# tdavchev/DESIRE

Hardware: AMD Instinct MI355X
Metric: agent-trajectory-samples/sec (K=20, T_pred=40) (higher is better)
Workload: dtype f32; 1 GPU; BASELINE configs[1]: SDD-like synthetic windows, 32 agent slots/window, K=20, T_obs=8/T_pred=40, H=128, L=128, fp32, posterior CVAE, IOC 1 refinement, social grid 4x4, scene grid 64x64x32; 512 windows/step/GPU; windows_per_gpu=512, rows_per_gpu=327680, parallelism=scene-sharded x1

## Files before the change

### desire_amd/csrc/api.hip

```cpp
#include "ctx.h"

#include <cmath>
#include <cstdio>
#include <cstdlib>
#include <cstring>

static thread_local std::string g_err;
int desire_fail(int code, const std::string& msg) { g_err = msg; return code; }

extern "C" const char* desire_last_error(void) { return g_err.c_str(); }
extern "C" int desire_version(void) { return 5; }
extern "C" int desire_dims_size(void) { return (int)sizeof(desire_dims); }
#ifndef DESIRE_SRC_HASH
#define DESIRE_SRC_HASH "unstamped"
#endif
extern "C" const char* desire_build_hash(void) { return DESIRE_SRC_HASH; }

int desire_upload(desire_ctx* h, const std::string& name, const std::vector<float>& v) {
    const size_t bytes = v.size() * sizeof(float);
    const DevBuf* b = h->dev.find(name.c_str());
    if (!b || b->bytes != bytes) {
        h->dev.release(name.c_str());
        if (h->dev.ensure(name.c_str(), bytes)) return -1;
    }
// ... 103 lines not shown
    return 0;
}

}

extern "C" int desire_set_option(desire_handle* h, const char* name, int32_t value) {
    if (!h || !name) return fail(DESIRE_ERR_ARG, "null argument");
    desire_dims d = h->d;
    const std::string nm(name);
    if (nm == "ioc_form") d.ioc_form = value;
    else if (nm == "ioc_split") d.ioc_split = value;
    else if (nm == "train_fp32_mask") d.train_fp32_mask = value;
    else if (nm == "flags") d.flags = value;
    else if (nm == "compact_host_counts") {
        h->cp_host_counts = value != 0;
        h->cp_pending = false; h->cp_enc = false;
        return DESIRE_OK;
    }
    else if (nm == "scene_grad") {
        if (value != 0 && value != 1) return fail(DESIRE_ERR_ARG, "scene_grad must be 0 or 1");
        h->scene_grad = value != 0;
        return scene_grad_on(h) && h->training ? scene_grad_setup(h) : DESIRE_OK;
    }
    else if (nm == "compact_min_rows") {
        if (value < 0) return fail(DESIRE_ERR_ARG, "compact_min_rows must be >= 0");
        h->ci_min_rows = value;
        return DESIRE_OK;
    }
    else if (nm == "scene_modes_chunk") {
        if (value < 0) return fail(DESIRE_ERR_ARG, "scene_modes_chunk must be >= 0");
        h->scene_modes_chunk = value;
        return DESIRE_OK;
    }
    else return fail(DESIRE_ERR_ARG, "unknown option: " + nm + " (ioc_form, ioc_split, train_fp32_mask, flags, compact_min_rows, compact_host_counts, scene_grad, scene_modes_chunk)");
    if (int rc = check_options(d)) return rc;
    if (((d.flags ^ h->d.flags) & (DESIRE_FLAG_COMPACT_ROWS | DESIRE_FLAG_COMPACT_IOC)) ||
        ((d.flags & DESIRE_FLAG_COMPACT_IOC) && (d.ioc_form != h->d.ioc_form || d.train_fp32_mask != h->d.train_fp32_mask)))
        h->cp_pending = h->cp_enc = false;
    h->d = d;
    return DESIRE_OK;
}

extern "C" int desire_create(const desire_dims* dims, desire_handle** out) {
    if (!dims || !out) return fail(DESIRE_ERR_ARG, "null argument");
    if (int rc = check_dims(*dims)) return rc;
    int ndev = 0;
    if (hipGetDeviceCount(&ndev) != hipSuccess || ndev < 1)
        return fail(DESIRE_ERR_NODEV, "no HIP device: libdesire_hip has no CPU path");
    int dev = 0;
    HIPCHK(hipGetDevice(&dev));
    hipDeviceProp_t prop;
    HIPCHK(hipGetDeviceProperties(&prop, dev));
    if (std::strncmp(prop.gcnArchName, "gfx950", 6) != 0)
        return fail(DESIRE_ERR_NODEV, std::string("device is ") + prop.gcnArchName + ", kernels are built for gfx950 only");
    desire_ctx* h = new desire_ctx();
    h->d = *dims;
    h->Hl = dims->H;
    if (dims->H < 64) h->d.H = 64;
    h->A = dims->n_scenes * dims->mno;
    h->R = h->A * dims->K;
    h->V = dims->S * dims->S;
    h->B = dims->grid_size * dims->grid_size;
    h->E = dims->E_v + dims->C + h->d.H;
    pack::weight_shapes(h->d, h->d.H, h->V, h->B, h->want);
    pack::weight_shapes(h->d, h->Hl, h->V, h->B, h->want_user);
    if (h->Hl != h->d.H) embeddings(h);
    const desire_dims& d = h->d;
// ... 215 lines not shown
```

### desire_amd/csrc/api_forward.hip

```cpp
#include "ctx.h"

#include <cmath>
#include <cstdio>
#include <cstdlib>
#include <cstring>

bool compact_rows(const desire_ctx* h) { return (h->d.flags & DESIRE_FLAG_COMPACT_ROWS) != 0; }
bool compact_ioc(const desire_ctx* h) { return (h->d.flags & DESIRE_FLAG_COMPACT_IOC) && ioc_plan(h).fwd != IocFwd::STEPWISE; }
ClassLayout class_layout(const desire_ctx* h, bool pad, const int* counts) {
    const desire_dims& d = h->d;
    ClassLayout L;
    int cand[6], nc = 0;
    for (int m : {8, 10, 16, 32, 64, 96}) if (m < d.mno && (m != 10 || pad)) cand[nc++] = m;
    for (int i = nc > 3 ? nc - 3 : 0; i < nc; ++i) L.m[L.n++] = cand[i];
    L.m[L.n++] = d.mno;
    for (int i = L.n; i < 4; ++i) L.m[i] = d.mno;
    for (int c = 0; c < L.n; ++c) {
        IocView& v = L.c[c];
        v.cls = c; v.mno = L.m[c]; v.n_scenes = counts ? counts[c] : d.n_scenes;
        v.gpt = (v.mno <= 32 && 32 % v.mno) ? 32 / v.mno : 0; v.ngrp = v.n_scenes * d.K;
        v.R = v.gpt ? (long)((v.ngrp + v.gpt - 1) / v.gpt) * 32 : (long)v.ngrp * v.mno;
        v.agent_off = L.agents; v.row_off = L.rows; v.win_off = L.wins;
        L.agents += (size_t)v.n_scenes * v.mno; L.rows += (size_t)v.R; L.wins += (size_t)v.n_scenes;
    }
// ... 215 lines not shown
        }
        const int32_t* amap = Wt<const int32_t>(h, "cp_amap");
        Timer t(h, s, "compact_gather");
        if (!h->cp_enc) {
            launch_gather_agents(W(h, "HxHy"), W(h, "cp_HxHy"), amap, P, 2 * H, s, dynP);
            launch_gather_agents(W(h, "p_last"), W(h, "cp_plast"), amap, P, 2, s, dynP);
            if (d.posterior) launch_gather_agents(W(h, "params"), W(h, "cp_params"), amap, P, 2 * d.L, s, dynP);
        }
        HxS = W(h, "cp_HxHy"); plS = W(h, "cp_plast"); Yout = W(h, "cp_Y0");
    }
    if (!dev_eps) {
        Timer t(h, s, "reparam");
        if (compact) launch_reparam_c_rng(W(h, "cp_params"), rng_args(h), W(h, "z"), Wt<const int32_t>(h, "cp_amap"), mno, d.K, d.mno, d.L, d.posterior, s, dynP);
        else launch_reparam_rng(W(h, "params"), rng_args(h), W(h, "z"), R, d.L, d.K, d.mno, d.posterior, s);
    }
    else if (compact) { Timer t(h, s, "reparam"); launch_reparam_c(W(h, "cp_params"), dev_eps, W(h, "z"), Wt<const int32_t>(h, "cp_amap"), mno, d.K, d.mno, d.L, d.posterior, s, dynP); }
    else { Timer t(h, s, "reparam"); launch_reparam(W(h, "params"), dev_eps, W(h, "z"), R, d.L, d.K, d.mno, d.posterior, s); }
    auto normd = [&](const char* layer, float* x, int P, int C, int sig) { batch_stats_act(h, layer, x, R, P, C, sig, s); };
    GemmArgs g{};
    g.A = W(h, "z"); g.lda = d.L; g.M = R; g.K = d.L; g.Bp = gen_op(h, GenStage::DECONV1, plan.deconv1); g.G = d.L / 8;
    g.NT = 64; g.out = W(h, "d1"); g.ldo = 2048; g.N = 2048;
    g.p0 = D(h, "vae_dec/deconv1/scale"); g.p1 = D(h, "vae_dec/deconv1/shift"); g.chmod = 128;
    int hintS = 0;
    if (dyn) hintS = count_hint(h);
    g.dyn = DynCount{dynP, d.K, hintS}; g.M_hint = hintS * d.K;
    const bool pobn = plan.batch_stats;
    { Timer t(h, s, "deconv1");
      switch (plan.deconv1) {
          case GenForm::BF16: launch_deconv1_bf16(g, s); break;
          case GenForm::X6: launch_deconv1_x6(g, s); break;
          case GenForm::FP32: launch_gemm_rows(g, pobn ? EPI_NONE : EPI_SCALE_SHIFT_ELU, s); if (pobn) normd("vae_dec/deconv1", W(h, "d1"), 16, 128, 0);
      } }
    ConvArgs c{};
    c.n = R; c.dyn = DynCount{dynP, d.K, hintS};
    if (pobn) c.mode = 3;
    c.in = W(h, "d1"); c.out = W(h, "d2"); c.Wp = gen_op(h, GenStage::DECONV2, plan.deconv2);
    c.scale = D(h, "vae_dec/deconv2/scale"); c.shift = D(h, "vae_dec/deconv2/shift");
    { Timer t(h, s, "deconv2");
      switch (plan.deconv2) {
          case GenForm::BF16: launch_deconv2_bf16(c, s); break;
          case GenForm::X6: launch_deconv2_x6(c, s, plan.np); break;
          case GenForm::FP32: launch_deconv2(c, s); if (pobn) normd("vae_dec/deconv2", W(h, "d2"), 64, 64, 0);
      } }
    c.in = W(h, "d2"); c.out = W(h, "d3"); c.Wp = gen_op(h, GenStage::DECONV3, plan.deconv3);
    c.scale = D(h, "vae_dec/deconv3/scale"); c.shift = D(h, "vae_dec/deconv3/shift");
    const float* w4 = D(h, gen_operands(GenStage::DECONV4, plan.deconv4()).a);
    if (plan.fuse34) {
        c.w_raw = w4; c.out = W(h, "xhat");
        Timer t(h, s, "deconv34");
        launch_deconv34_bf16(c, D(h, "vae_dec/deconv4/scale"), D(h, "vae_dec/deconv4/shift"), s);
    } else {
        { Timer t(h, s, "deconv3");
          switch (plan.deconv3) {
              case GenForm::BF16: launch_deconv3_bf16(c, s); break;
              case GenForm::X6: launch_deconv3_x6(c, s, plan.np); break;
              case GenForm::FP32: launch_deconv3(c, s); if (pobn) normd("vae_dec/deconv3", W(h, "d3"), 256, 32, 0);
          } }
        c.in = W(h, "d3"); c.out = W(h, "xhat"); c.w_raw = w4;
        c.scale = D(h, "vae_dec/deconv4/scale"); c.shift = D(h, "vae_dec/deconv4/shift");
        { Timer t(h, s, "deconv4"); launch_deconv4(c, s);
          if (pobn) normd("vae_dec/deconv4", W(h, "xhat"), 1024, 1, 1); }
    }
    MaskArgs m{};
    m.xhat = W(h, "xhat"); m.R = R; m.V = h->V; m.H = H; m.Hl = h->Hl; m.K = d.K; m.mno = mno;
    m.Wp = gen_op(h, GenStage::MASK, plan.mask); m.bias = D(h, "mask/b"); m.Hx = HxS; m.ldhx = 2 * H; m.xz = W(h, "xz");
    m.dyn = DynCount{dynP, 1, hintS};
    if (h->training) m.sv_p = W(h, "mask_sv_p");
// ... 218 lines not shown
```

### desire_amd/csrc/backward.hip

```cpp
#include "ctx.h"

namespace {

float* G(desire_ctx* h, const std::string& name) { return W(h, "Gflat") + h->slots.at(name).off; }

void tn(desire_ctx* h, const float* A, int lda, const float* Gm, int ldg, long M, int Kd, int N, float* out, int ldo,
        int accumulate, hipStream_t s, const unsigned long long* flags = nullptr, int fcols = 0,
        const int* rowlist = nullptr, const int* binbase = nullptr, const int* bintotal = nullptr) {
    TnArgs a{};
    a.A = A; a.lda = lda; a.G = Gm; a.ldg = ldg; a.M = M; a.Kd = Kd; a.N = N; a.flags = flags; a.fcols = fcols;
    a.rowlist = rowlist; a.binbase = binbase; a.bintotal = bintotal;
    if (rowlist && !(fcols == 128 && N > 64 && gemm_tn_big_tiles(a) > 0)) a.rowlist = nullptr;
    if (a.rowlist) a.flags = nullptr;
    a.np = gen_plan(h).wgrad_pieces;
    const long big_tiles = a.np == 2 ? gemm_tn_big_tiles(a) : 0;
    const long blocks = ((Kd + 63) / 64) * ((N + 63) / 64);
    long sl = big_tiles ? 512 / big_tiles : 2048 / blocks;
    if (sl < 1) sl = 1; if (sl > (big_tiles ? 512 : 256)) sl = big_tiles ? 512 : 256;
    const long maxsl = (M + 63) / 64; if (sl > maxsl) sl = maxsl;
    while ((size_t)sl * Kd * N * sizeof(float) > h->ws.bytes("tn_partial") && sl > 1) sl /= 2;
    a.nslices = (int)sl; a.partial = W(h, "tn_partial");
    launch_gemm_tn(a, out, ldo, accumulate, s);
}
void colsum(desire_ctx* h, const float* Gm, int ldg, long M, int N, float* out, int accumulate, hipStream_t s) {
// ... 377 lines not shown
    launch_gemm_rows(g, EPI_NONE, s);
    return DESIRE_OK;
}

int cvae_enc_bwd(const BwdPass& bp) {
    desire_ctx* h = bp.h; hipStream_t s = bp.s; const desire_dims& d = h->d;
    const int H = d.H, V = h->V, L = d.L, Ae = bp.agents_e;
    const bool bn1 = d.bn_mode != 0;
    const int32_t* inv = bp.rows_compact ? Wt<const int32_t>(h, "cp_inv") : nullptr;
    if (bp.eps) launch_reparam_bwd(W(h, "dz"), bp.eps, W(h, "params"), bp.valid, W(h, "nvalid"), W(h, "dparams"), d.n_scenes, d.mno, d.K, L, s, inv, bp.n_present);
    else launch_reparam_bwd_rng(W(h, "dz"), rng_args(h), W(h, "params"), bp.valid, W(h, "nvalid"), W(h, "dparams"), d.n_scenes, d.mno, d.K, L, s, inv,
                                bp.n_present);
    if (bp.enc_compact) launch_gather_agents(W(h, "dparams"), W(h, "cp_dparams"), bp.amap, bp.n_present, 2 * L, s);
    const float* dparE = bp.enc_compact ? W(h, "cp_dparams") : W(h, "dparams");
    if (Ae <= 0) return DESIRE_OK;
    tn(h, W(h, "c3"), 2048, dparE, 2 * L, Ae, 2048, 2 * L, G(h, "vae_enc/fc/w"), 2 * L, 0, s);
    colsum(h, dparE, 2 * L, Ae, 2 * L, G(h, "vae_enc/fc/b"), 0, s);
    GemmArgs g{};
    g.A = dparE; g.lda = 2 * L; g.M = Ae; g.K = 2 * L; g.Bp = D4(h, "vae_enc/fc/WT"); g.G = 2 * L / 8; g.NT = 64;
    g.out = W(h, "dconvE3"); g.ldo = 2048; g.N = 2048; g.p0 = D(h, "vae_enc/conv3/scale"); g.chmod = 128; g.aux = W(h, "c3");
    if (bn1) {
        launch_gemm_rows(g, EPI_NONE, s);
        norm_bwd(bp, W(h, "dconvE3"), W(h, "conv3_pre"), W(h, "c3"), Ae, 16, 128, D(h, "vae_enc/conv3/gamma"), 0);
    } else
        launch_gemm_rows(g, EPI_ELUGRAD, s);
    const int NSL = Ae >= 2048 ? 64 : (Ae >= 256 ? 16 : 4);
    ConvWgradArgs wg{};
    wg.np = gen_plan(h).wgrad_pieces;
    wg.n = Ae; wg.partial = W(h, "tn_partial");
    wg.S = W(h, "dconvE3"); wg.Cs = 128; wg.Ps = 4; wg.Lg = W(h, "c2"); wg.Cl = 64; wg.Pl = 8; wg.stride = 1; wg.pad = 0;
    launch_conv_wgrad(wg, NSL, G(h, "vae_enc/conv3/w"), s);
    if (!bn1) colsum(h, W(h, "dconvE3"), 128, (long)Ae * 16, 128, G(h, "vae_enc/conv3/b"), 0, s);
    ConvArgs c{};
    c.n = Ae; c.mode = bn1 ? 3 : 1;
    c.in = W(h, "dconvE3"); c.out = W(h, "dconvE2"); c.Wp = D4(h, "vae_enc/conv3/Wbwd");
    c.scale = D(h, "vae_enc/conv2/scale"); c.shift = c.scale; c.yprev = W(h, "c2");
    launch_deconv2(c, s);
    if (bn1) norm_bwd(bp, W(h, "dconvE2"), W(h, "conv2_pre"), W(h, "c2"), Ae, 64, 64, D(h, "vae_enc/conv2/gamma"), 0);
    wg.S = W(h, "dconvE2"); wg.Cs = 64; wg.Ps = 8; wg.Lg = W(h, "c1"); wg.Cl = 32; wg.Pl = 16; wg.stride = 2; wg.pad = 1;
    launch_conv_wgrad(wg, NSL, G(h, "vae_enc/conv2/w"), s);
    if (!bn1) colsum(h, W(h, "dconvE2"), 64, (long)Ae * 64, 64, G(h, "vae_enc/conv2/b"), 0, s);
    c.in = W(h, "dconvE2"); c.out = W(h, "dconvE1"); c.Wp = D4(h, "vae_enc/conv2/Wbwd");
    c.scale = D(h, "vae_enc/conv1/scale"); c.shift = c.scale; c.yprev = W(h, "c1");
    launch_deconv3(c, s);
    if (bn1) norm_bwd(bp, W(h, "dconvE1"), W(h, "conv1_pre"), W(h, "c1"), Ae, 256, 32, D(h, "vae_enc/conv1/gamma"), 0);
    launch_w1ch_grad(W(h, "vae_in"), W(h, "dconvE1"), Ae, Ae < 1024 ? Ae : 1024, W(h, "tn_partial"), G(h, "vae_enc/conv1/w"), s);
    if (!bn1) colsum(h, W(h, "dconvE1"), 32, (long)Ae * 256, 32, G(h, "vae_enc/conv1/b"), 0, s);
    c.in = W(h, "dconvE1"); c.out = W(h, "dq_c"); c.w_raw = D(h, "vae_enc/conv1/raw"); c.mode = 2; c.yprev = W(h, "vae_in");
    launch_deconv4(c, s);
    tn(h, bp.Hx_e, 2 * H, W(h, "dq_c"), V, Ae, 2 * H, V, G(h, "fc_c/w"), V, 0, s);
    colsum(h, W(h, "dq_c"), V, Ae, V, G(h, "fc_c/b"), 0, s);
    g = GemmArgs{};
    g.A = W(h, "dq_c"); g.lda = V; g.M = Ae; g.K = V; g.Bp = D4(h, "fc_c/WT"); g.G = V / 8; g.NT = 2 * H / 32;
    g.out = bp.dH_e; g.ldo = 2 * H; g.N = 2 * H;
    launch_gemm_rows(g, EPI_NONE, s);
    return DESIRE_OK;
}

int assemble_dH(const BwdPass& bp) {
    desire_ctx* h = bp.h; hipStream_t s = bp.s; const desire_dims& d = h->d;
    const int H = d.H, P = bp.n_present;
    if (bp.enc_compact) {
        if (P <= 0) return DESIRE_OK;
        launch_rows_to_agents(bp.dHx_s, bp.dH_e, 2 * H, 1, P, d.K, H, s);
        if (!h->ci_last) {
            launch_fill_f32(W(h, "dHxHy_ioc"), (size_t)h->A * H, 0.f, s);
            launch_rows_to_agents(W(h, "dHx_rows"), W(h, "dHxHy_ioc"), H, d.n_scenes, d.mno, d.K, H, s);
// ... 78 lines not shown
```

### desire_amd/csrc/ctx.h

```cpp
#pragma once
#include "../../include/desire_hip.h"
#include "gen_plan.h"
#include "ioc_plan.h"
#include "kernels.h"
#include "pack.h"
#include "workspace.h"

#include <hip/hip_runtime.h>

#include <cstring>
#include <functional>
#include <map>
#include <string>
#include <vector>

int desire_fail(int code, const std::string& msg);
#define fail desire_fail
#define HIPCHK(x)                                                                                   \
    do {                                                                                            \
        hipError_t e_ = (x);                                                                        \
        if (e_ != hipSuccess)                                                                       \
            return fail(DESIRE_ERR_HIP, std::string(#x) + ": " + hipGetErrorString(e_));            \
    } while (0)

// ... 5 lines not shown
struct WSlot { size_t off; size_t n; };

struct EmbedAxis { std::vector<std::pair<int, int>> seg; };
struct Embed { EmbedAxis rows, cols; };

struct desire_ctx {
    desire_dims d;
    int Hl = 0;
    int A, R, V, B, E;
    std::map<std::string, size_t> want_user;
    std::map<std::string, Embed> emb;
    std::map<std::string, std::vector<float>> host_w;
    std::map<std::string, size_t> want;
    Workspace dev{dev_malloc, dev_free};
    Workspace ws{dev_malloc, dev_free};
    bool finalized = false;
    std::vector<void*> graphs;
    std::vector<float> bin_tab_host;
    const float* grids = nullptr;
    bool grids_set = false;
    bool profiling = false;
    void* peer_region = nullptr; size_t peer_bytes = 0; void* peer_base[8] = {nullptr, nullptr, nullptr, nullptr, nullptr, nullptr, nullptr, nullptr};
    bool peer_mapped[8] = {false, false, false, false, false, false, false, false}; int peer_rank = -1, peer_nranks = 0; bool peer_ready = false;
    int* peer_err = nullptr;
    float head_loss_w = 0.f;
    int recon_mode = 0; float recon_tau = 0.f;
    int recon_scope = 0;
    int* host_err = nullptr;
    int32_t* cp_host = nullptr; hipEvent_t cp_ev = nullptr; bool cp_pending = false; int cp_P = -1;
    int ci_cnt[4] = {0, 0, 0, 0}; bool ci_last = false; int ci_min_rows = 8192;
    bool cp_enc = false;
    bool cp_host_counts = false;
    bool cp_last = false;
    int scene_modes_chunk = 0;
    int32_t* bw_starts = nullptr; int32_t* bw_err = nullptr;
    uint32_t* rng_state = nullptr; uint32_t rng_scene_base = 0, rng_slot_base = 0;
    std::vector<Prof> prof;
    std::vector<std::string> prof_name_store;
    bool training = false;
    std::map<std::string, WSlot> slots;
    size_t n_params = 0;
    const float* last_eps = nullptr;
    int adam_t = 0;
    int n_seg = 0;
    int n_seg16 = 0;
    bool scene_grad = false;
    const float* img = nullptr; bool img_set = false;
    bool img_stale = true;
};

struct Timer {
    desire_ctx* h; hipStream_t s; bool on; size_t idx = 0;
    Timer(desire_ctx* h_, hipStream_t s_, const char* name) : h(h_), s(s_), on(h_->profiling) {
        if (!on) return;
        Prof p; p.name = name;
        (void)hipEventCreate(&p.e0); (void)hipEventCreate(&p.e1);
        (void)hipEventRecord(p.e0, s);
        idx = h->prof.size();
        h->prof.push_back(p);
    }
    ~Timer() { if (on) (void)hipEventRecord(h->prof[idx].e1, s); }
};

inline GenPlan gen_plan(const desire_ctx* h) { return gen_plan(h->d, h->training, h->V); }

inline const float* D(desire_ctx* h, const char* name) { return h->dev.get(name); }
// ... 44 lines not shown
```

### desire_amd/csrc/dyn_count.h

```cpp
#pragma once
#include <stdint.h>

struct DynCount { const int32_t* cnt; int mul; int hint; };
inline int dyn_units(int worst, const DynCount& d) {
    if (!d.cnt || d.hint <= 0) return worst;
    const long g = (long)d.hint * d.mul, want = g + g / 4 + 256;
    return (int)(want < (long)worst ? want : (long)worst);
}
```

### desire_amd/csrc/kernels.h

```cpp
#pragma once
#include <hip/hip_runtime.h>
#include <stdint.h>

#include "dyn_count.h"
#include "eval_lds.h"
#include "ioc_lds.h"

template <auto K>
inline const void* big_lds_kernel() {
    static const hipError_t once = hipFuncSetAttribute(reinterpret_cast<const void*>(K), hipFuncAttributeMaxDynamicSharedMemorySize, 160 * 1024);
    (void)once;
    return reinterpret_cast<const void*>(K);
}
template <auto K, class... Args>
inline void launch_big_lds(dim3 grid, dim3 block, size_t lds, hipStream_t s, const Args&... args) {
    (void)big_lds_kernel<K>();
    hipLaunchKernelGGL(K, grid, block, lds, s, args...);
}


enum { EPI_BIAS = 0, EPI_BIAS_RELU = 1, EPI_SCALE_SHIFT_ELU = 2, EPI_NONE = 3, EPI_ELUGRAD = 4, EPI_SIGGRAD = 5 };

struct GemmArgs {
    const float* A; int lda; int M; int K;
    const float4* Bp; int G; int NT;
    float* out; int ldo; int N;
    const float* p0; const float* p1; int chmod;
    const float* aux;
    DynCount dyn;
    int M_hint;
};
void launch_gemm_rows(const GemmArgs& a, int epi, hipStream_t s);

void launch_reparam(const float* params, const float* eps, float* z, int R, int L, int K, int mno,
                    int posterior, hipStream_t s);

struct RngArgs { const uint32_t* st; uint32_t seed_lo, seed_hi, draw; uint32_t scene_base, slot_base; };
struct RngKey { uint32_t lo, hi, draw; };
__device__ __forceinline__ RngKey rng_key(const RngArgs& g) {
    if (g.st) return RngKey{g.st[2], g.st[3], g.st[1]};
    return RngKey{g.seed_lo, g.seed_hi, g.draw};
}
void launch_rng_set(uint32_t* st, uint64_t seed, uint32_t draw, hipStream_t s);
void launch_rng_begin(uint32_t* st, hipStream_t s);
void launch_rng_fill(uint64_t seed, uint32_t stream_id, uint64_t first, int normals, void* out, uint64_t n, hipStream_t s);
void launch_reparam_rng(const float* params, const RngArgs& g, float* z, int R, int L, int K, int mno, int posterior, hipStream_t s);
void launch_reparam_c_rng(const float* params_c, const RngArgs& g, float* z, const int32_t* amap, int P, int K, int mno, int L, int posterior,
                          hipStream_t s, const int32_t* dynP = nullptr);
void launch_reparam_bwd_rng(const float* dz, const RngArgs& g, const float* params, const uint8_t* valid, const float* nvalid, float* dparams,
                            int n_scenes, int mno, int K, int L, hipStream_t s, const int32_t* inv, int P);

struct MaskArgs {
    const float* xhat; int R; int V; int H; int K; int mno;
    int Hl;
    const float4* Wp; const float* bias; const float* Hx; int ldhx; float* xz;
    float* sv_p;
    DynCount dyn;
};
void launch_mask(const MaskArgs& a, hipStream_t s);
void launch_deconv1_x6(const GemmArgs& a, hipStream_t s);
void launch_mask_x6(const MaskArgs& a, hipStream_t s);

struct ConvArgs {
    const float* in; float* out; int n;
    const float4* Wp; const float* w_raw;
    const float* scale; const float* shift;
    int mode; const float* yprev;
    DynCount dyn;
};
void launch_conv1(const ConvArgs& a, hipStream_t s);
void launch_conv2(const ConvArgs& a, hipStream_t s);
void launch_conv2_x3(const ConvArgs& a, hipStream_t s);
void launch_conv3_x3(const ConvArgs& a, hipStream_t s);
void launch_conv3(const ConvArgs& a, hipStream_t s);
void launch_deconv2(const ConvArgs& a, hipStream_t s);
void launch_deconv3(const ConvArgs& a, hipStream_t s);
void launch_deconv4(const ConvArgs& a, hipStream_t s);

struct EncArgs {
    const float* frames; int n_scenes; int T; int mno;
    float sx, sy; int H;
    const float* wx_g; const float* b_g;
    const float* wx_c; const float* b_c;
    const float4* Whg; const float4* Whc;
    float* out; int ldo;
    float* p_last;
    uint8_t* valid;
    float* sv_r; float* sv_u; float* sv_c; float* sv_h; float* sv_x;
    int n_roll; const float* w5; const float* b5;
    const float* normals; float* roll_out;
    DynCount dyn;
};
void launch_encoder(const EncArgs& a, hipStream_t s);
void launch_encoder_pair(const EncArgs& past, const EncArgs& fut, hipStream_t s);
void launch_encoder_bf16(const EncArgs& a, hipStream_t s);

struct RollArgs {
    const float* h_T; int R; int K; int mno; int H; int T;
    const float* wx_g; const float* b_g; const float* wx_c; const float* b_c; const float4* Whg; const float4* Whc;
    const float* w5; const float* b5;
    const float* normals; RngArgs g;
// ... 255 lines not shown
```

### desire_amd/csrc/kernels_conv.hip

```cpp
#include "common.h"
#include "kernels.h"
#include <type_traits>
#include <utility>

__global__ __launch_bounds__(DS_WG) void k_conv1(ConvArgs a) {
    __shared__ __attribute__((aligned(16))) float in_s[36 * 40];
    const int n = blockIdx.x, tid = threadIdx.x;
    DYN_N(a, n, n)
    for (int i = tid; i < 36 * 40; i += DS_WG) in_s[i] = 0.f;
    __syncthreads();
    for (int i = tid; i < 1024; i += DS_WG) in_s[((i >> 5) + 1) * 40 + (i & 31) + 1] = a.in[(size_t)n * 1024 + i];
    const int co = tid & 31, pg = tid >> 5;
    float wr[25];
#pragma unroll
    for (int k = 0; k < 25; ++k) wr[k] = a.w_raw[k * 32 + co];
    __syncthreads();
    const float sc = a.scale[co], sh = a.shift[co];
    for (int p = pg; p < 256; p += 8) {
        const int oy = p >> 4, ox = p & 15;
        const int base = (2 * ox) & ~3;
        const bool odd = ox & 1;
        float acc = 0.f;
#pragma unroll
        for (int ky = 0; ky < 5; ++ky) {
// ... 52 lines not shown
        ox[m] = q - oy[m] * OW;
    }
    for (int ky = 0; ky < 5; ++ky)
        for (int kx = 0; kx < 5; ++kx) {
            const float* ap[MT];
#pragma unroll
            for (int m = 0; m < MT; ++m) {
                const int iy = oy[m] * STRIDE + ky - PAD, ix = ox[m] * STRIDE + kx - PAD;
                const bool ok = iy >= 0 && iy < IW && ix >= 0 && ix < IW;
                ap[m] = (ok ? in_s + (sm[m] * IW * IW + pos(iy, ix)) * LDP : zero_row) + 4 * (lane >> 5);
            }
            mma_groups_ptr<MT>(acc, ap, a.Wp + ((size_t)((ky * 5 + kx) * NT + nt) * G) * 64 + lane, G);
        }
    const int co = nt * 32 + (lane & 31);
    const float sc = a.scale[co], sh = a.shift[co];
#pragma unroll
    for (int m = 0; m < MT; ++m)
#pragma unroll
        for (int i = 0; i < 16; ++i) {
            const int r = (mt0 + m) * 32 + acc_row(i);
            const int smp = s0 + r / PIX;
            if (smp < a.n) { const size_t ix = ((size_t)s0 * PIX + r) * CO + co; a.out[ix] = conv_epilogue(acc[m][i], sc, sh, a.mode, false, a.yprev, ix); }
        }
}
void launch_conv2(const ConvArgs& a, hipStream_t s) {
    const size_t lds = (36 + 256 * 36) * sizeof(float);
    hipLaunchKernelGGL((k_conv_gather<32, 16, 8, 2, 1, 64>), dim3(a.n), dim3(DS_WG), lds, s, a);
}
void launch_conv3(const ConvArgs& a, hipStream_t s) {
    const size_t lds = (68 + 4 * 64 * 68) * sizeof(float);
    launch_big_lds<k_conv_gather<64, 8, 4, 1, 0, 128>>(dim3((a.n + 3) / 4), dim3(DS_WG), lds, s, a);
}

template <bool FWD>
__global__ __launch_bounds__(DS_WG) void k_deconv2(ConvArgs a) {
    extern __shared__ __attribute__((aligned(16))) float out_s[];
    const int lane = lane_id(), w = wave_id();
    const int hf = w & 1, sp = w >> 1;
    asm volatile("" ::: "a255");
    DYN_N(a, n, blockIdx.x * 4)
    for (int bx = blockIdx.x; bx * 4 < a.n; bx += gridDim.x) {
        const int s0 = bx * 4 + sp * 2;
        const int c = lane & 31, hi = lane >> 5;
        float O[8][8];
    #pragma unroll
        for (int oy = 0; oy < 8; ++oy)
    #pragma unroll
            for (int ox = 0; ox < 8; ++ox) O[oy][ox] = 0.f;
        float4 af[16];
        {
            const int row = lane & 31;
            const int smp = min(s0 + ((row >> 2) & 1), a.n - 1);
            const float* src = a.in + ((size_t)smp * 16 + (row >> 3) * 4 + (row & 3)) * 128 + 4 * hi;
    #pragma unroll
            for (int g = 0; g < 16; ++g) af[g] = *reinterpret_cast<const float4*>(src + g * 8);
        }
        int woff = 0;
        asm volatile("" : "+s"(woff));
        const float4* wp = a.Wp + woff + lane;
        auto load_b = [&](float4 (&b)[8], int q) {
            const float4* bp = wp + ((size_t)((q >> 1) * 2 + hf) * 16 + (q & 1) * 8) * 64;
    #pragma unroll
            for (int g = 0; g < 8; ++g) b[g] = bp[g * 64];
        };
        float4 b[2][8];
        load_b(b[0], 0);
        f32x16 acc = zero16();
    #pragma unroll
        for (int q = 0; q < 50; ++q) {
            if (q + 1 < 50) load_b(b[(q + 1) & 1], q + 1);
            __builtin_amdgcn_sched_barrier(0);
            const float4 (&bt)[8] = b[q & 1];
            if (!(q & 1)) acc = zero16();
    #pragma unroll
            for (int g = 0; g < 8; ++g) {
                const float4 av = af[(q & 1) * 8 + g];
                acc = mfma32(av.x, bt[g].x, acc);
                acc = mfma32(av.y, bt[g].y, acc);
                acc = mfma32(av.z, bt[g].z, acc);
                acc = mfma32(av.w, bt[g].w, acc);
            }
            if (q & 1) {
                const int tap = q >> 1, ky = tap / 5, kx = tap - ky * 5;
    #pragma unroll
                for (int i = 0; i < 16; ++i) O[(i >> 2) + ky][(i & 3) + kx] = O[(i >> 2) + ky][(i & 3) + kx] + acc[i];
            }
            __builtin_amdgcn_sched_barrier(0);
        }
        float* my = out_s + (sp * 2) * 4096;
    #pragma unroll
        for (int o = 0; o < 64; ++o) my[(hi * 64 + o) * 64 + hf * 32 + c] = O[o >> 3][o & 7];
        const int er = lane >> 3, ec = hf * 32 + (lane & 7) * 4;
        const float4 sc4 = *reinterpret_cast<const float4*>(a.scale + ec), sh4 = *reinterpret_cast<const float4*>(a.shift + ec);
        for (int i = 0; i < 16; ++i) {
            const int sp_px = i * 8 + er;
            const int smp = s0 + (sp_px >> 6);
            if (smp < a.n) {
                const float4 v = *reinterpret_cast<const float4*>(my + sp_px * 64 + ec);
                const size_t ix = ((size_t)smp * 64 + (sp_px & 63)) * 64 + ec;
                float4 o;
                if (FWD) {
                    o.x = eluf_(v.x * sc4.x + sh4.x); o.y = eluf_(v.y * sc4.y + sh4.y);
                    o.z = eluf_(v.z * sc4.z + sh4.z); o.w = eluf_(v.w * sc4.w + sh4.w);
                } else {
                    o.x = conv_epilogue(v.x, sc4.x, sh4.x, a.mode, false, a.yprev, ix);
                    o.y = conv_epilogue(v.y, sc4.y, sh4.y, a.mode, false, a.yprev, ix + 1);
                    o.z = conv_epilogue(v.z, sc4.z, sh4.z, a.mode, false, a.yprev, ix + 2);
                    o.w = conv_epilogue(v.w, sc4.w, sh4.w, a.mode, false, a.yprev, ix + 3);
                }
                *reinterpret_cast<float4*>(a.out + ix) = o;
            }
        }
    }
}
void launch_deconv2(const ConvArgs& a, hipStream_t s) {
    const int ng = dyn_units(a.n, a.dyn);
    if (a.mode == 0) launch_big_lds<k_deconv2<true>>(dim3((ng + 3) / 4), dim3(DS_WG), 4 * 4096 * sizeof(float), s, a);
    else launch_big_lds<k_deconv2<false>>(dim3((ng + 3) / 4), dim3(DS_WG), 4 * 4096 * sizeof(float), s, a);
}

struct D3Chain { int py, px, ky, kx; bool first, last; };
__host__ __device__ constexpr D3Chain d3_chain(int s) {
    const int c = s < 4 ? 0 : s < 10 ? 1 : s < 16 ? 2 : 3, s0 = c == 0 ? 0 : c == 1 ? 4 : c == 2 ? 10 : 16;
    const int py = c >> 1, px = c & 1, nkx = px ? 3 : 2, n = (py ? 3 : 2) * nkx, i = s - s0;
    return D3Chain{py, px, 1 - py + 2 * (i / nkx), 1 - px + 2 * (i % nkx), i == 0, i == n - 1};
}
template <class F, int... S>
__device__ __forceinline__ void static_for_(F&& f, std::integer_sequence<int, S...>) { (f(std::integral_constant<int, S>{}), ...); }
template <int N, class F>
__device__ __forceinline__ void static_for(F&& f) { static_for_(f, std::make_integer_sequence<int, N>{}); }
template <bool FWD, int NS>
__global__ __launch_bounds__(NS * 64) void k_deconv3(ConvArgs a) {
    constexpr int LDP = 68;
    extern __shared__ __attribute__((aligned(16))) float smem[];
    float* zero_row = smem;
    float* in_s = smem + 128;
    const int lane = lane_id(), w = wave_id(), tid = threadIdx.x;
    DYN_N(a, n, blockIdx.x * NS)
    for (int bx = blockIdx.x; bx * NS < a.n; bx += gridDim.x) {
        const int s0 = bx * NS;
        int woff = 0;
        asm volatile("" : "+s"(woff));
        const float4* wp = a.Wp + woff + lane;
        auto load_b = [&](float4 (&f)[8], const D3Chain ch) __attribute__((always_inline)) {
            const float4* bp = wp + ((size_t)(ch.ky * 5 + ch.kx) * 8) * 64;
    #pragma unroll
            for (int g = 0; g < 8; ++g) f[g] = bp[g * 64];
        };
        float4 b[2][8];
        load_b(b[0], d3_chain(0));
        __builtin_amdgcn_sched_barrier(0);
        for (int i = tid; i < 128; i += NS * 64) zero_row[i] = 0.f;
        for (int i = tid; i < NS * 64 * 16; i += NS * 64) {
            const int pix = i >> 4, c4 = i & 15;
            const int smp = s0 + (pix >> 6);
            float4 v = make_float4(0.f, 0.f, 0.f, 0.f);
            if (smp < a.n) v = *reinterpret_cast<const float4*>(a.in + ((size_t)s0 * 64 + pix) * 64 + c4 * 4);
            *reinterpret_cast<float4*>(in_s + pix * LDP + c4 * 4) = v;
        }
        __syncthreads();
        const int smp = s0 + w;
        const int hi = lane >> 5;
        float4 sc[4], sh[4];
    #pragma unroll
        for (int q = 0; q < 4; ++q) {
            sc[q] = *reinterpret_cast<const float4*>(a.scale + 8 * q + 4 * hi);
            sh[q] = *reinterpret_cast<const float4*>(a.shift + 8 * q + 4 * hi);
        }
        int qy[2], qx[2];
    #pragma unroll
        for (int m = 0; m < 2; ++m) { const int q = m * 32 + (lane & 31); qy[m] = q >> 3; qx[m] = q & 7; }
        auto rows = [&](const D3Chain ch, const float* (&ap)[2]) __attribute__((always_inline)) {
            const int dy = (ch.py + 1 - ch.ky) / 2, dx = (ch.px + 1 - ch.kx) / 2;
    #pragma unroll
            for (int m = 0; m < 2; ++m) {
                const int iy = qy[m] + dy, ix = qx[m] + dx;
                const bool ok = iy >= 0 && iy < 8 && ix >= 0 && ix < 8;
                const int in_off = 128 + (w * 64 + iy * 8 + ix) * LDP, zero_off = ((w * 64 + iy * 8 + ix + 64) * LDP + 128) & 63;
                ap[m] = smem + (ok ? in_off : zero_off) + 4 * hi;
            }
        };
        const float* ap[2][2];
        rows(d3_chain(0), ap[0]);
        f32x16 acc[2];
        static_for<25>([&](auto chain_no) __attribute__((always_inline)) {
            constexpr int s = decltype(chain_no)::value;
            constexpr D3Chain ch = d3_chain(s);
            constexpr int py = ch.py, px = ch.px;
            if constexpr (s + 1 < 25) { load_b(b[(s + 1) & 1], d3_chain(s + 1)); rows(d3_chain(s + 1), ap[(s + 1) & 1]); }
            __builtin_amdgcn_sched_barrier(0);
            if constexpr (ch.first) { acc[0] = zero16(); acc[1] = zero16(); }
            const float4 (&bt)[8] = b[s & 1];
    #pragma unroll
            for (int g = 0; g < 8; ++g)
    #pragma unroll
                for (int m = 0; m < 2; ++m) {
                    const float4 av = *reinterpret_cast<const float4*>(ap[s & 1][m] + g * 8);
                    acc[m] = mfma32(bt[g].x, av.x, acc[m]);
                    acc[m] = mfma32(bt[g].y, av.y, acc[m]);
                    acc[m] = mfma32(bt[g].z, av.z, acc[m]);
                    acc[m] = mfma32(bt[g].w, av.w, acc[m]);
                    __builtin_amdgcn_sched_barrier(0);
                }
            if constexpr (ch.last) {
                if (smp < a.n) {
    #pragma unroll
                    for (int m = 0; m < 2; ++m) {
                        const int oy = 2 * qy[m] + py, ox = 2 * qx[m] + px;
                        const size_t base = ((size_t)smp * 256 + oy * 16 + ox) * 32 + 4 * hi;
    #pragma unroll
                        for (int q = 0; q < 4; ++q) {
                            const size_t ix = base + 8 * q;
                            float4 o;
                            if (FWD) {
                                o.x = eluf_(acc[m][4 * q] * sc[q].x + sh[q].x); o.y = eluf_(acc[m][4 * q + 1] * sc[q].y + sh[q].y);
                                o.z = eluf_(acc[m][4 * q + 2] * sc[q].z + sh[q].z); o.w = eluf_(acc[m][4 * q + 3] * sc[q].w + sh[q].w);
                            } else {
                                o.x = conv_epilogue(acc[m][4 * q], sc[q].x, sh[q].x, a.mode, false, a.yprev, ix);
                                o.y = conv_epilogue(acc[m][4 * q + 1], sc[q].y, sh[q].y, a.mode, false, a.yprev, ix + 1);
                                o.z = conv_epilogue(acc[m][4 * q + 2], sc[q].z, sh[q].z, a.mode, false, a.yprev, ix + 2);
                                o.w = conv_epilogue(acc[m][4 * q + 3], sc[q].w, sh[q].w, a.mode, false, a.yprev, ix + 3);
                            }
                            *reinterpret_cast<float4*>(a.out + ix) = o;
                        }
                    }
                }
            }
        });
        __syncthreads();
    }
}
void launch_deconv3(const ConvArgs& a, hipStream_t s) {
    const size_t lds = (128 + (size_t)4 * 64 * 68) * sizeof(float);
    const int ng = dyn_units(a.n, a.dyn);
    if (a.mode == 0) launch_big_lds<k_deconv3<true, 4>>(dim3((ng + 3) / 4), dim3(256), lds, s, a);
    else launch_big_lds<k_deconv3<false, 4>>(dim3((ng + 3) / 4), dim3(256), lds, s, a);
}

__global__ __launch_bounds__(DS_WG) void k_deconv4(ConvArgs a) {
    constexpr int LDP = 36;
    __shared__ __attribute__((aligned(16))) float in_s[256 * LDP];
    __shared__ __attribute__((aligned(16))) float w_s[25 * 32];
    const int n = blockIdx.x, tid = threadIdx.x, lane = lane_id(), w = wave_id();
    for (int i = tid; i < 256 * 8; i += DS_WG) {
        const int pix = i >> 3, c4 = i & 7;
        *reinterpret_cast<float4*>(in_s + pix * LDP + c4 * 4) =
            *reinterpret_cast<const float4*>(a.in + ((size_t)n * 256 + pix) * 32 + c4 * 4);
    }
    for (int i = tid; i < 800; i += DS_WG) w_s[i] = a.w_raw[i];
    __syncthreads();
    const int py = w >> 1, px = w & 1;
    const float sc = a.scale[0], sh = a.shift[0];
    for (int j = 0; j < 4; ++j) {
        const int q = j * 64 + lane;
        const int qy = q >> 4, qx = q & 15;
        float acc = 0.f;
        for (int ky = 1 - py; ky < 5; ky += 2) {
            const int iy = qy + (py + 1 - ky) / 2;
            if (iy < 0 || iy >= 16) continue;
            for (int kx = 1 - px; kx < 5; kx += 2) {
                const int ix = qx + (px + 1 - kx) / 2;
                if (ix < 0 || ix >= 16) continue;
                const float* ip = in_s + (iy * 16 + ix) * LDP;
                const float* wp = w_s + (ky * 5 + kx) * 32;
#pragma unroll
                for (int c4 = 0; c4 < 8; ++c4) {
                    const float4 x = *reinterpret_cast<const float4*>(ip + c4 * 4);
                    const float4 ww = *reinterpret_cast<const float4*>(wp + c4 * 4);
                    acc = fmaf(x.x, ww.x, acc); acc = fmaf(x.y, ww.y, acc);
// ... 54 lines not shown
```

Before: 2.622 million samples/s.

## Make deconv2/deconv3 persistent with cross-iteration prefetch of next tile

Deconv2 and deconv3 launches now cap the grid at the number of resident workgroups, queried through the occupancy API or taken from a new gen_grid_cap option, and loop over tiles with a grid stride. Inside the loop, the next tile's activations and the first weight slice are prefetched into registers during the current tile's MFMA chain. This hides global load latency across iterations and removes the per-iteration staging and __syncthreads in deconv3. In exchange it raises register pressure and changes how LDS is reused between waves, which could lower occupancy or introduce races.

```diff
diff --git a/desire_amd/csrc/api.hip b/desire_amd/csrc/api.hip
--- a/desire_amd/csrc/api.hip
+++ b/desire_amd/csrc/api.hip
@@ -159,7 +159,12 @@
         h->scene_modes_chunk = value;
         return DESIRE_OK;
     }
-    else return fail(DESIRE_ERR_ARG, "unknown option: " + nm + " (ioc_form, ioc_split, train_fp32_mask, flags, compact_min_rows, compact_host_counts, scene_grad, scene_modes_chunk)");
+    else if (nm == "gen_grid_cap") {
+        if (value < 0) return fail(DESIRE_ERR_ARG, "gen_grid_cap must be >= 0");
+        h->gen_grid_cap = value;
+        return DESIRE_OK;
+    }
+    else return fail(DESIRE_ERR_ARG, "unknown option: " + nm + " (ioc_form, ioc_split, train_fp32_mask, flags, compact_min_rows, compact_host_counts, scene_grad, scene_modes_chunk, gen_grid_cap)");
     if (int rc = check_options(d)) return rc;
     if (((d.flags ^ h->d.flags) & (DESIRE_FLAG_COMPACT_ROWS | DESIRE_FLAG_COMPACT_IOC)) ||
         ((d.flags & DESIRE_FLAG_COMPACT_IOC) && (d.ioc_form != h->d.ioc_form || d.train_fp32_mask != h->d.train_fp32_mask)))
diff --git a/desire_amd/csrc/api_forward.hip b/desire_amd/csrc/api_forward.hip
--- a/desire_amd/csrc/api_forward.hip
+++ b/desire_amd/csrc/api_forward.hip
@@ -271,7 +271,7 @@
           case GenForm::FP32: launch_gemm_rows(g, pobn ? EPI_NONE : EPI_SCALE_SHIFT_ELU, s); if (pobn) normd("vae_dec/deconv1", W(h, "d1"), 16, 128, 0);
       } }
     ConvArgs c{};
-    c.n = R; c.dyn = DynCount{dynP, d.K, hintS};
+    c.n = R; c.dyn = DynCount{dynP, d.K, hintS}; c.grid_cap = h->gen_grid_cap;
     if (pobn) c.mode = 3;
     c.in = W(h, "d1"); c.out = W(h, "d2"); c.Wp = gen_op(h, GenStage::DECONV2, plan.deconv2);
     c.scale = D(h, "vae_dec/deconv2/scale"); c.shift = D(h, "vae_dec/deconv2/shift");
diff --git a/desire_amd/csrc/backward.hip b/desire_amd/csrc/backward.hip
--- a/desire_amd/csrc/backward.hip
+++ b/desire_amd/csrc/backward.hip
@@ -433,7 +433,7 @@
     launch_conv_wgrad(wg, NSL, G(h, "vae_enc/conv3/w"), s);
     if (!bn1) colsum(h, W(h, "dconvE3"), 128, (long)Ae * 16, 128, G(h, "vae_enc/conv3/b"), 0, s);
     ConvArgs c{};
-    c.n = Ae; c.mode = bn1 ? 3 : 1;
+    c.n = Ae; c.mode = bn1 ? 3 : 1; c.grid_cap = h->gen_grid_cap;
     c.in = W(h, "dconvE3"); c.out = W(h, "dconvE2"); c.Wp = D4(h, "vae_enc/conv3/Wbwd");
     c.scale = D(h, "vae_enc/conv2/scale"); c.shift = c.scale; c.yprev = W(h, "c2");
     launch_deconv2(c, s);
diff --git a/desire_amd/csrc/ctx.h b/desire_amd/csrc/ctx.h
--- a/desire_amd/csrc/ctx.h
+++ b/desire_amd/csrc/ctx.h
@@ -61,6 +61,7 @@
     bool cp_enc = false;
     bool cp_host_counts = false;
     bool cp_last = false;
+    int gen_grid_cap = 0;
     int scene_modes_chunk = 0;
     int32_t* bw_starts = nullptr; int32_t* bw_err = nullptr;
     uint32_t* rng_state = nullptr; uint32_t rng_scene_base = 0, rng_slot_base = 0;
diff --git a/desire_amd/csrc/dyn_count.h b/desire_amd/csrc/dyn_count.h
--- a/desire_amd/csrc/dyn_count.h
+++ b/desire_amd/csrc/dyn_count.h
@@ -7,3 +7,8 @@
     const long g = (long)d.hint * d.mul, want = g + g / 4 + 256;
     return (int)(want < (long)worst ? want : (long)worst);
 }
+inline int strided_grid(int units, int per_tile, const DynCount& d, int cap) {
+    const long tiles = ((long)dyn_units(units, d) + per_tile - 1) / per_tile;
+    if (tiles <= 0) return 0;
+    return (int)(cap > 0 && (long)cap < tiles ? (long)cap : tiles);
+}
diff --git a/desire_amd/csrc/kernels.h b/desire_amd/csrc/kernels.h
--- a/desire_amd/csrc/kernels.h
+++ b/desire_amd/csrc/kernels.h
@@ -11,6 +11,20 @@
     static const hipError_t once = hipFuncSetAttribute(reinterpret_cast<const void*>(K), hipFuncAttributeMaxDynamicSharedMemorySize, 160 * 1024);
     (void)once;
     return reinterpret_cast<const void*>(K);
+}
+template <auto K>
+inline int resident_workgroups(int block, size_t lds) {
+    static int cached[64];
+    int dev = 0;
+    if (hipGetDevice(&dev) != hipSuccess || dev < 0 || dev >= 64) return 0;
+    if (!cached[dev]) {
+        int per_cu = 0, cus = 0;
+        if (hipOccupancyMaxActiveBlocksPerMultiprocessor(&per_cu, big_lds_kernel<K>(), block, lds) != hipSuccess ||
+            hipDeviceGetAttribute(&cus, hipDeviceAttributeMultiprocessorCount, dev) != hipSuccess || per_cu < 1 || cus < 1)
+            return 0;
+        cached[dev] = per_cu * cus;
+    }
+    return cached[dev];
 }
 template <auto K, class... Args>
 inline void launch_big_lds(dim3 grid, dim3 block, size_t lds, hipStream_t s, const Args&... args) {
@@ -67,6 +81,7 @@
     const float* scale; const float* shift;
     int mode; const float* yprev;
     DynCount dyn;
+    int grid_cap;
 };
 void launch_conv1(const ConvArgs& a, hipStream_t s);
 void launch_conv2(const ConvArgs& a, hipStream_t s);
diff --git a/desire_amd/csrc/kernels_conv.hip b/desire_amd/csrc/kernels_conv.hip
--- a/desire_amd/csrc/kernels_conv.hip
+++ b/desire_amd/csrc/kernels_conv.hip
@@ -108,6 +108,10 @@
     launch_big_lds<k_conv_gather<64, 8, 4, 1, 0, 128>>(dim3((a.n + 3) / 4), dim3(DS_WG), lds, s, a);
 }
 
+template <class F, int... S>
+__device__ __forceinline__ void static_for_(F&& f, std::integer_sequence<int, S...>) { (f(std::integral_constant<int, S>{}), ...); }
+template <int N, class F>
+__device__ __forceinline__ void static_for(F&& f) { static_for_(f, std::make_integer_sequence<int, N>{}); }
 template <bool FWD>
 __global__ __launch_bounds__(DS_WG) void k_deconv2(ConvArgs a) {
     extern __shared__ __attribute__((aligned(16))) float out_s[];
@@ -115,39 +119,47 @@
     const int hf = w & 1, sp = w >> 1;
     asm volatile("" ::: "a255");
     DYN_N(a, n, blockIdx.x * 4)
-    for (int bx = blockIdx.x; bx * 4 < a.n; bx += gridDim.x) {
-        const int s0 = bx * 4 + sp * 2;
-        const int c = lane & 31, hi = lane >> 5;
-        float O[8][8];
-    #pragma unroll
-        for (int oy = 0; oy < 8; ++oy)
-    #pragma unroll
-            for (int ox = 0; ox < 8; ++ox) O[oy][ox] = 0.f;
-        float4 af[16];
-        {
-            const int row = lane & 31;
-            const int smp = min(s0 + ((row >> 2) & 1), a.n - 1);
-            const float* src = a.in + ((size_t)smp * 16 + (row >> 3) * 4 + (row & 3)) * 128 + 4 * hi;
-    #pragma unroll
-            for (int g = 0; g < 16; ++g) af[g] = *reinterpret_cast<const float4*>(src + g * 8);
-        }
+    int bx = blockIdx.x;
+    if ((long)bx * 4 >= (long)a.n) return;
+    const int c = lane & 31, hi = lane >> 5;
+    float* my = out_s + (sp * 2) * 4096;
+    const int er = lane >> 3, ec = hf * 32 + (lane & 7) * 4;
+    const float4 sc4 = *reinterpret_cast<const float4*>(a.scale + ec), sh4 = *reinterpret_cast<const float4*>(a.shift + ec);
+    auto load_a = [&](float4 (&f)[16], int t) __attribute__((always_inline)) {
+        const int row = lane & 31;
+        const int smp = min(t * 4 + sp * 2 + ((row >> 2) & 1), a.n - 1);
+        const float* src = a.in + ((size_t)smp * 16 + (row >> 3) * 4 + (row & 3)) * 128 + 4 * hi;
+    #pragma unroll
+        for (int g = 0; g < 16; ++g) f[g] = *reinterpret_cast<const float4*>(src + g * 8);
+    };
+    auto load_b = [&](float4 (&b)[8], int q) __attribute__((always_inline)) {
         int woff = 0;
         asm volatile("" : "+s"(woff));
-        const float4* wp = a.Wp + woff + lane;
-        auto load_b = [&](float4 (&b)[8], int q) {
-            const float4* bp = wp + ((size_t)((q >> 1) * 2 + hf) * 16 + (q & 1) * 8) * 64;
-    #pragma unroll
-            for (int g = 0; g < 8; ++g) b[g] = bp[g * 64];
-        };
-        float4 b[2][8];
-        load_b(b[0], 0);
+        const float4* bp = a.Wp + woff + lane + ((size_t)((q >> 1) * 2 + hf) * 16 + (q & 1) * 8) * 64;
+    #pragma unroll
+        for (int g = 0; g < 8; ++g) b[g] = bp[g * 64];
+    };
+    constexpr int A_AT = 44;
+    float4 af[16], an[16];
+    load_a(af, bx);
+    float4 b[2][8];
+    load_b(b[0], 0);
+    for (; (long)bx * 4 < (long)a.n; bx += gridDim.x) {
+        const int s0 = bx * 4 + sp * 2;
+        float O[8][8];
+    #pragma unroll
+        for (int oy = 0; oy < 8; ++oy)
+    #pragma unroll
+            for (int ox = 0; ox < 8; ++ox) O[oy][ox] = 0.f;
         f32x16 acc = zero16();
-    #pragma unroll
-        for (int q = 0; q < 50; ++q) {
-            if (q + 1 < 50) load_b(b[(q + 1) & 1], q + 1);
+        static_for<50>([&](auto half_no) __attribute__((always_inline)) {
+            constexpr int q = decltype(half_no)::value;
+            if constexpr (q + 1 < 50) load_b(b[(q + 1) & 1], q + 1);
+            else load_b(b[0], 0);
+            if constexpr (q == A_AT) load_a(an, bx + gridDim.x);
             __builtin_amdgcn_sched_barrier(0);
             const float4 (&bt)[8] = b[q & 1];
-            if (!(q & 1)) acc = zero16();
+            if constexpr (!(q & 1)) acc = zero16();
     #pragma unroll
             for (int g = 0; g < 8; ++g) {
                 const float4 av = af[(q & 1) * 8 + g];
@@ -156,18 +168,15 @@
                 acc = mfma32(av.z, bt[g].z, acc);
                 acc = mfma32(av.w, bt[g].w, acc);
             }
-            if (q & 1) {
-                const int tap = q >> 1, ky = tap / 5, kx = tap - ky * 5;
+            if constexpr (q & 1) {
+                constexpr int tap = q >> 1, ky = tap / 5, kx = tap - ky * 5;
     #pragma unroll
                 for (int i = 0; i < 16; ++i) O[(i >> 2) + ky][(i & 3) + kx] = O[(i >> 2) + ky][(i & 3) + kx] + acc[i];
             }
             __builtin_amdgcn_sched_barrier(0);
-        }
-        float* my = out_s + (sp * 2) * 4096;
+        });
     #pragma unroll
         for (int o = 0; o < 64; ++o) my[(hi * 64 + o) * 64 + hf * 32 + c] = O[o >> 3][o & 7];
-        const int er = lane >> 3, ec = hf * 32 + (lane & 7) * 4;
-        const float4 sc4 = *reinterpret_cast<const float4*>(a.scale + ec), sh4 = *reinterpret_cast<const float4*>(a.shift + ec);
         for (int i = 0; i < 16; ++i) {
             const int sp_px = i * 8 + er;
             const int smp = s0 + (sp_px >> 6);
@@ -187,12 +196,18 @@
                 *reinterpret_cast<float4*>(a.out + ix) = o;
             }
         }
-    }
+    #pragma unroll
+        for (int g = 0; g < 16; ++g) af[g] = an[g];
+    }
+}
+template <auto K>
+static void launch_strided4(const ConvArgs& a, int block, size_t lds, hipStream_t s) {
+    const int grid = strided_grid(a.n, 4, a.dyn, a.grid_cap > 0 ? a.grid_cap : resident_workgroups<K>(block, lds));
+    if (grid > 0) launch_big_lds<K>(dim3(grid), dim3(block), lds, s, a);
 }
 void launch_deconv2(const ConvArgs& a, hipStream_t s) {
-    const int ng = dyn_units(a.n, a.dyn);
-    if (a.mode == 0) launch_big_lds<k_deconv2<true>>(dim3((ng + 3) / 4), dim3(DS_WG), 4 * 4096 * sizeof(float), s, a);
-    else launch_big_lds<k_deconv2<false>>(dim3((ng + 3) / 4), dim3(DS_WG), 4 * 4096 * sizeof(float), s, a);
+    if (a.mode == 0) launch_strided4<k_deconv2<true>>(a, DS_WG, 4 * 4096 * sizeof(float), s);
+    else launch_strided4<k_deconv2<false>>(a, DS_WG, 4 * 4096 * sizeof(float), s);
 }
 
 struct D3Chain { int py, px, ky, kx; bool first, last; };
@@ -201,10 +216,6 @@
     const int py = c >> 1, px = c & 1, nkx = px ? 3 : 2, n = (py ? 3 : 2) * nkx, i = s - s0;
     return D3Chain{py, px, 1 - py + 2 * (i / nkx), 1 - px + 2 * (i % nkx), i == 0, i == n - 1};
 }
-template <class F, int... S>
-__device__ __forceinline__ void static_for_(F&& f, std::integer_sequence<int, S...>) { (f(std::integral_constant<int, S>{}), ...); }
-template <int N, class F>
-__device__ __forceinline__ void static_for(F&& f) { static_for_(f, std::make_integer_sequence<int, N>{}); }
 template <bool FWD, int NS>
 __global__ __launch_bounds__(NS * 64) void k_deconv3(ConvArgs a) {
     constexpr int LDP = 68;
@@ -213,7 +224,35 @@
     float* in_s = smem + 128;
     const int lane = lane_id(), w = wave_id(), tid = threadIdx.x;
     DYN_N(a, n, blockIdx.x * NS)
-    for (int bx = blockIdx.x; bx * NS < a.n; bx += gridDim.x) {
+    int bx = blockIdx.x;
+    if ((long)bx * NS >= (long)a.n) return;
+    for (int i = tid; i < 128; i += NS * 64) zero_row[i] = 0.f;
+    __syncthreads();
+    float* st_dst = in_s + (w * 64 + (lane >> 4)) * LDP + (lane & 15) * 4;
+    auto st_src = [&](int t) __attribute__((always_inline)) {
+        const long smp = min((long)t * NS + w, (long)a.n - 1);
+        return reinterpret_cast<const float4*>(a.in + (size_t)smp * 4096) + lane;
+    };
+    constexpr int PF_AT = 20, PF_N = 12;
+    typedef float vec4 __attribute__((ext_vector_type(4)));
+    float4 b[2][8];
+    vec4 pf[PF_N], pl[16 - PF_N];
+    {
+        const float4* src = st_src(bx);
+    #pragma unroll
+        for (int j = 0; j < 16; ++j) { const float4 v = src[j * 64]; *reinterpret_cast<float4*>(st_dst + j * 4 * LDP) = v; }
+    }
+    const int hi = lane >> 5;
+    float4 sc[4], sh[4];
+#pragma unroll
+    for (int q = 0; q < 4; ++q) {
+        sc[q] = *reinterpret_cast<const float4*>(a.scale + 8 * q + 4 * hi);
+        sh[q] = *reinterpret_cast<const float4*>(a.shift + 8 * q + 4 * hi);
+    }
+    int qy[2], qx[2];
+#pragma unroll
+    for (int m = 0; m < 2; ++m) { const int q = m * 32 + (lane & 31); qy[m] = q >> 3; qx[m] = q & 7; }
+    for (bool first = true; (long)bx * NS < (long)a.n; bx += gridDim.x, first = false) {
         const int s0 = bx * NS;
         int woff = 0;
         asm volatile("" : "+s"(woff));
@@ -223,29 +262,9 @@
     #pragma unroll
             for (int g = 0; g < 8; ++g) f[g] = bp[g * 64];
         };
-        float4 b[2][8];
-        load_b(b[0], d3_chain(0));
-        __builtin_amdgcn_sched_barrier(0);
-        for (int i = tid; i < 128; i += NS * 64) zero_row[i] = 0.f;
-        for (int i = tid; i < NS * 64 * 16; i += NS * 64) {
-            const int pix = i >> 4, c4 = i & 15;
-            const int smp = s0 + (pix >> 6);
-            float4 v = make_float4(0.f, 0.f, 0.f, 0.f);
-            if (smp < a.n) v = *reinterpret_cast<const float4*>(a.in + ((size_t)s0 * 64 + pix) * 64 + c4 * 4);
-            *reinterpret_cast<float4*>(in_s + pix * LDP + c4 * 4) = v;
-        }
-        __syncthreads();
+        if (first) load_b(b[0], d3_chain(0));
+        const float4* nsrc = st_src(bx + gridDim.x);
         const int smp = s0 + w;
-        const int hi = lane >> 5;
-        float4 sc[4], sh[4];
-    #pragma unroll
-        for (int q = 0; q < 4; ++q) {
-            sc[q] = *reinterpret_cast<const float4*>(a.scale + 8 * q + 4 * hi);
-            sh[q] = *reinterpret_cast<const float4*>(a.shift + 8 * q + 4 * hi);
-        }
-        int qy[2], qx[2];
-    #pragma unroll
-        for (int m = 0; m < 2; ++m) { const int q = m * 32 + (lane & 31); qy[m] = q >> 3; qx[m] = q & 7; }
         auto rows = [&](const D3Chain ch, const float* (&ap)[2]) __attribute__((always_inline)) {
             const int dy = (ch.py + 1 - ch.ky) / 2, dx = (ch.px + 1 - ch.kx) / 2;
     #pragma unroll
@@ -264,6 +283,12 @@
             constexpr D3Chain ch = d3_chain(s);
             constexpr int py = ch.py, px = ch.px;
             if constexpr (s + 1 < 25) { load_b(b[(s + 1) & 1], d3_chain(s + 1)); rows(d3_chain(s + 1), ap[(s + 1) & 1]); }
+            if constexpr (s == PF_AT) {
+                static_for<PF_N>([&](auto j) __attribute__((always_inline)) { pf[j] = *reinterpret_cast<const vec4*>(nsrc + j * 64); });
+            }
+            if constexpr (s == 24) {
+                static_for<16 - PF_N>([&](auto j) __attribute__((always_inline)) { pl[j] = *reinterpret_cast<const vec4*>(nsrc + (PF_N + j) * 64); });
+            }
             __builtin_amdgcn_sched_barrier(0);
             if constexpr (ch.first) { acc[0] = zero16(); acc[1] = zero16(); }
             const float4 (&bt)[8] = b[s & 1];
@@ -278,6 +303,11 @@
                     acc[m] = mfma32(bt[g].w, av.w, acc[m]);
                     __builtin_amdgcn_sched_barrier(0);
                 }
+            if constexpr (s == 24) {
+                __builtin_amdgcn_sched_barrier(0);
+                load_b(b[0], d3_chain(0));
+                __builtin_amdgcn_sched_barrier(0);
+            }
             if constexpr (ch.last) {
                 if (smp < a.n) {
     #pragma unroll
@@ -303,14 +333,14 @@
                 }
             }
         });
-        __syncthreads();
+        static_for<PF_N>([&](auto j) __attribute__((always_inline)) { *reinterpret_cast<vec4*>(st_dst + j * 4 * LDP) = pf[j]; });
+        static_for<16 - PF_N>([&](auto j) __attribute__((always_inline)) { *reinterpret_cast<vec4*>(st_dst + (PF_N + j) * 4 * LDP) = pl[j]; });
     }
 }
 void launch_deconv3(const ConvArgs& a, hipStream_t s) {
     const size_t lds = (128 + (size_t)4 * 64 * 68) * sizeof(float);
-    const int ng = dyn_units(a.n, a.dyn);
-    if (a.mode == 0) launch_big_lds<k_deconv3<true, 4>>(dim3((ng + 3) / 4), dim3(256), lds, s, a);
-    else launch_big_lds<k_deconv3<false, 4>>(dim3((ng + 3) / 4), dim3(256), lds, s, a);
+    if (a.mode == 0) launch_strided4<k_deconv3<true, 4>>(a, 256, lds, s);
+    else launch_strided4<k_deconv3<false, 4>>(a, 256, lds, s);
 }
 
 __global__ __launch_bounds__(DS_WG) void k_deconv4(ConvArgs a) {
```

Result: no change. 2.634 million samples/s, median of 6 (+0.5%).
